# amberxie88/latent_diffusion_planning

Measured on AMD Instinct MI355X. Metric: latent plans/sec (horizon=9, 100 DDIM steps), higher is better.
Workload: dtype f32; 1 GPU; configs[1]: rm_lift planner ConditionalUnet1D (D=25, T=8, down_dims [256,512,1024]), 100-step DDIM, batch 256 synthetic latents per GPU, random-init weights, Philox noise, hipGraph-captured loop; plans_per_gpu=256, denoise_steps=100, sampler=ddim, graph=True, parallelism=dp1, ranks_seen_by_backend=1, backend=none, range_fallback=0, fp16_plane_launches=0

## Files before the change

### latent_diffusion_planning_amd/csrc/engine.hip

```cpp
#include "engine.hpp"
#include "sconv.hpp"
#include "t2pack.hpp"
#include "t4pack.hpp"
#include "version.h"

#include <algorithm>
#include <cmath>
#include <cstring>

namespace ldp {

void betas_squaredcos(int n, std::vector<float>& betas, std::vector<float>& alphas,
                             std::vector<float>& acp) {
  auto abar = [](double t) {
    const double c = std::cos((t + 0.008) / 1.008 * M_PI / 2.0);
    return c * c;
  };
  betas.resize(n);
  alphas.resize(n);
  acp.resize(n);
  float run = 1.0f;
  for (int i = 0; i < n; ++i) {
    const double b = std::min(1.0 - abar((double)(i + 1) / n) / abar((double)i / n), 0.999);
    betas[i] = (float)b;
// ... 1572 lines not shown
  return agent_sample_impl(h, obs_emb, obs_frames, obs_horizon, x_init, x_noise, a_init, a_noise, seed, row_offset, sampler, planner_steps,
                           idm_steps, x_out, plan_out, action_out, act_lo, act_hi, act_dim, act_mode, B, use_graph, stream, nullptr, &cs);
}

int ldp_agent_sample_guided(ldp_handle* h, const float* obs_emb, int32_t obs_frames, int32_t obs_horizon, const float* x_init,
                            const float* x_noise, const float* a_init, const float* a_noise, const float* target, const float* wg,
                            const float* anchor, const float* lam, const float* beta, const float* lo, const float* hi, const float* rho,
                            int32_t n_rho, uint64_t seed, int64_t row_offset, int32_t sampler, int32_t planner_steps, int32_t idm_steps,
                            float* x_out, float* plan_out, float* action_out, const float* act_lo, const float* act_hi, int32_t act_dim,
                            int32_t act_mode, int32_t B, int32_t use_graph, void* stream) {
  const GuideSpec gd{target, wg, anchor, lam, beta, lo, hi, rho, n_rho};
  return agent_sample_impl(h, obs_emb, obs_frames, obs_horizon, x_init, x_noise, a_init, a_noise, seed, row_offset, sampler, planner_steps,
                           idm_steps, x_out, plan_out, action_out, act_lo, act_hi, act_dim, act_mode, B, use_graph, stream, nullptr, nullptr,
                           &gd);
}

int ldp_policy_sample(ldp_handle* h, const float* obs_emb, int32_t obs_frames, int32_t obs_horizon, int32_t img_width,
                      const float* x_init, const float* x_noise, uint64_t seed, int64_t row_offset, int32_t sampler, int32_t n_steps,
                      float* action_out, const float* act_lo, const float* act_hi, int32_t act_dim, int32_t act_mode,
                      int32_t B, int32_t use_graph, void* stream) {
  if (!h || !obs_emb || !action_out || B <= 0) return fail(LDP_EINVAL, "bad argument");
  if (!h->pl.ready) return fail(LDP_ESTATE, "planner weights not finalized");
  PlannerState& P = h->pl;
  const int ah = h->cfg.action_horizon, A = P.D;
  if (obs_horizon <= 0 || obs_frames < obs_horizon || P.G <= 0 || P.G % obs_horizon != 0)
    return fail(LDP_EINVAL, "obs_horizon %d does not divide global_cond_dim %d (frames given: %d)", obs_horizon, P.G, obs_frames);
  const int E = P.G / obs_horizon;
  if (img_width < 0 || img_width > E) return fail(LDP_EINVAL, "img_width %d must lie in 0..%d (the per-frame width)", img_width, E);
  if (ah < 1 || ah > P.T) return fail(LDP_EINVAL, "action_horizon %d must be in 1..pred_horizon %d", ah, P.T);
  if (act_dim != 0 && (act_dim != 1 && act_dim != A)) return fail(LDP_EINVAL, "action bounds of length %d (A = %d)", act_dim, A);
  if (act_dim != 0 && (!act_lo || !act_hi)) return fail(LDP_EINVAL, "action bounds missing");
  if (!x_noise) {
    if (const int b1 = batch_split(h, B)) {
      const size_t xr = (size_t)P.T * A, ar = (size_t)ah * A;
      LDP_TRY(ldp_policy_sample(h, obs_emb, obs_frames, obs_horizon, img_width, x_init, nullptr, seed, row_offset, sampler, n_steps,
                                action_out, act_lo, act_hi, act_dim, act_mode, b1, use_graph, stream));
      const int64_t c1 = h->last_conv_launches, t1 = h->last_total_launches;
      const int r2 = ldp_policy_sample(h, obs_emb + (size_t)b1 * obs_frames * E, obs_frames, obs_horizon, img_width,
                                       x_init ? x_init + b1 * xr : nullptr, nullptr, seed, row_offset + b1, sampler, n_steps,
                                       action_out + b1 * ar, act_lo, act_hi, act_dim, act_mode, B - b1, use_graph, stream);
      h->last_conv_launches += c1; h->last_total_launches += t1;
      return r2;
    }
  }
  LDP_TRY(check_sampler(sampler, n_steps, P.n_train, "planner", h));
  LDP_TRY(entry_fault_check(h));
  hipStream_t s = (hipStream_t)stream;
  LDP_TRY(planner_workspace(h, B));
  h->last_conv_launches = h->last_total_launches = 0;
  LoopSpec L{n_steps, sampler, x_noise != nullptr && sampler == LDP_SAMPLER_DDPM, 0, n_steps};
  LDP_TRY(planner_pre(h, nullptr, x_init, x_noise, seed, row_offset, L, B, s));
  LDP_TRY(gather_dp_cond_launch(obs_emb, P.cond.f(), B, obs_frames, E, obs_horizon, img_width, s));
  const int Bg = bucket_rows(B, L.explicit_noise);
  GraphKey key{0, Bg, n_steps, sampler, L.explicit_noise ? 1 : 0, 0, 0, 0, n_steps};
  LDP_TRY(run_or_replay(h, key, use_graph != 0, s, [&](hipStream_t q) { return planner_loop(h, Bg, L, q); }));
  LDP_TRY(head_rows_launch(P.state.f(), action_out, B, P.T, ah, A, P.DP, s));
  if (act_dim != 0) LDP_TRY(normalize_launch(action_out, action_out, (int64_t)B * ah * A, act_lo, act_hi, act_dim, act_mode, s));
  return LDP_OK;
}

int ldp_normalize_bounds(const float* x, float* y, int64_t n, const float* lo, const float* hi,
                         int32_t dim, int32_t normalize, void* stream) {
  if (!x || !y || !lo || !hi || dim <= 0) return fail(LDP_EINVAL, "bad argument");
  return normalize_launch(x, y, n, lo, hi, dim, normalize, (hipStream_t)stream);
}

int ldp_mean_sq_diff(const float* a, const float* b, int64_t n, float* out, void* stream) {
  if (!a || !b || !out || n <= 0) return fail(LDP_EINVAL, "bad argument");
  return mean_sq_diff_launch(a, b, n, out, (hipStream_t)stream);
}

int ldp_reduce_stats(const float* x, int64_t n, float* out4, void* stream) {
  if (!x || !out4 || n <= 0) return fail(LDP_EINVAL, "bad argument");
  return reduce_stats_launch(x, n, out4, (hipStream_t)stream);
}

int ldp_add_noise(const float* x0, const float* noise, const int32_t* t_dev, int32_t n_train, float* out, int64_t rows,
                  int32_t width, void* stream) {
  if (!x0 || !noise || !t_dev || !out || rows <= 0 || width <= 0) return fail(LDP_EINVAL, "bad argument");
  if (n_train < 1 || n_train > 256) return fail(LDP_EINVAL, "n_train must be in 1..256 (the abar table travels by value), got %d", n_train);
  std::vector<float> betas, alphas, acp;
  betas_squaredcos(n_train, betas, alphas, acp);
  AbarTable tab{};
  std::copy(acp.begin(), acp.end(), tab.v);
  return add_noise_launch(x0, noise, t_dev, tab, n_train, out, rows, width, (hipStream_t)stream);
}

int ldp_check_fault(ldp_handle* h, void* stream) {
  if (!h) return fail(LDP_EINVAL, "null handle");
  LDP_HIP(hipStreamSynchronize((hipStream_t)stream));
  reap_retired_graphs(h);
  int32_t f = 0;
  LDP_TRY(ldp_poll_fault(h, &f));
  if (f & 1)
    return fail(LDP_EFAULT, "a split work-group timed out waiting for its peer: the results enqueued since the "
                "previous check are invalid (the handle now runs in safe mode; re-issue the calls)");
  if (f & 2)
    return fail(LDP_EFAULT, "an operand left the range of the two-fp16-plane form (|x| >= 65504): the results enqueued since the "
                "previous check are invalid (the handle now runs its split convolutions on three bf16 planes; re-issue the calls)");
  return LDP_OK;
}

int ldp_poll_fault(ldp_handle* h, int32_t* faulted) {
  if (!h || !faulted) return fail(LDP_EINVAL, "bad argument");
  const int f = h->fault_pending | take_faults(h);
  h->fault_pending = 0;
  *faulted = f;
  return LDP_OK;
}

int ldp_set_option(ldp_handle* h, const char* name, int64_t value) {
  if (!h || !name) return fail(LDP_EINVAL, "bad argument");
  const std::string n(name);
  Options& o = h->opt;
  const int v = (int)value;
  if (n == "no_csplit") o.no_csplit = v;
  else if (n == "no_mb2") o.no_mb2 = v;
  else if (n == "no_kw") o.no_kw = v;
  else if (n == "kw_min_it") o.kw_min_it = v;
  else if (n == "kw_bmax") o.kw_bmax = v;
  else if (n == "no_fin_rows") o.no_fin_rows = v;
  else if (n == "no_batch_split") o.no_batch_split = v;
  else if (n == "up_full_depth") o.up_full_depth = v;
  else if (n == "planner_split") o.planner_split = v;
  else if (n == "planner_split_updown") o.planner_split_updown = v;
  else if (n == "planner_split_cs2") o.planner_split_cs2 = v;
  else if (n == "planner_split_c256") o.planner_split_c256 = v;
  else if (n == "planner_split_mb2") o.planner_split_mb2 = v;
  else if (n == "planner_split_t2res") o.planner_split_t2res = v;
  else if (n == "planner_split_t16") o.planner_split_t16 = v;
  else if (n == "planner_split_f16") o.planner_split_f16 = v;
  else if (n == "vae_no_conv_stats") o.vae_no_conv_stats = v;
  else if (n == "vae_no_conv_in_stats") o.vae_no_conv_in_stats = v;
  else if (n == "vae_split") o.vae_split = v;
  else if (n == "vae_split_f16") o.vae_split_f16 = v;
  else if (n == "vae_split_gn_only") o.vae_split_gn_only = v;
  else if (n == "vae_split_s2") o.vae_split_s2 = v;
  else if (n == "graph_cap") { h->graph_cap = v; return LDP_OK; }
  else if (n == "timeline_ptr") o.timeline_ptr = value;
  else if (n == "idm_unfused") o.idm_unfused = v;
  else if (n == "idm_rt_major") o.idm_rt_major = v;
  else if (n == "idm_noring") o.idm_noring = v;
  else if (n == "idm_stream") o.idm_stream = v;
  else if (n == "by_sample") o.by_sample = v;
  else if (n == "place2d") { o.place2d = v; drop_graphs(h); }
  else if (n == "idm_f16") o.idm_f16 = v;
  else if (n == "idm_f16_min_rows") o.idm_f16_min_rows = v < 32 ? 32 : v;
  else if (n == "idm_f16_hs") o.idm_f16_hs = v;
  else if (n == "train_small_wg") o.train_small_wg = v;
  else if (n == "train_big") o.train_big = v;
  else if (n == "train_split") o.train_split = v;
  else if (n == "train_streams") o.train_streams = v;
  else if (n == "train_intra_split") o.train_intra_split = v;
  else if (n == "train_group_proj") o.train_group_proj = v;
  else if (n == "train_gn4") o.train_gn4 = v;
  else if (n == "train_sides") o.train_sides = v;
  else if (n == "train_fuse_reduce") o.train_fuse_reduce = v;
  else if (n == "train_wg_target") o.train_wg_target = v;
  else if (n == "idm_hs") { if (v != 0 && v != 1 && v != 2 && v != 4 && v != 8) return fail(LDP_EINVAL, "idm_hs must be 0, 1, 2, 4 or 8"); o.idm_hs = v; }
  else if (n == "dbg" || n == "repeat") {
#ifdef LDP_ABLATE
    if (n == "dbg") o.dbg = v; else o.repeat = v < 1 ? 1 : v;
#else
    if (!(n == "dbg" ? v == 0 : v == 1))
      return fail(LDP_EINVAL, "option '%s': the timing ablations are compiled into libldp_hip_abl.so only (make -C csrc ablate; tools take it with --lib)", name);
#endif
  }
  else if (n == "t2_mb2") o.t2_mb2 = v;
  else if (n == "planner_split_t2all16") o.planner_split_t2all16 = v;
  else if (n == "planner_split_t2res16") o.planner_split_t2res16 = v;
  else if (n == "planner_split_8w") o.planner_split_8w = v;
  else if (n == "safe_mode") h->safe_mode = v != 0;
  else if (n == "range_fallback") h->range_fallback = v != 0;
  else if (n == "dump_plans") {
    std::map<std::string, int64_t> text = v == 2 ? tconv_plan_log() : std::map<std::string, int64_t>();
    if (v != 2) for (const auto& kv : h->plan_log) text[plan_text(kv.first)] = kv.second;
    for (const auto& kv : text) fprintf(stderr, "PLAN %s launches=%lld\n", kv.first.c_str(), (long long)kv.second);
    return LDP_OK;
  }
  else if (n == "inject_fault") { if (v && h->fault_host) h->fault_host[v == 2 ? 1 : 0] = 1u; return LDP_OK; }
  else return fail(LDP_EKEY, "unknown option '%s'", name);
  drop_graphs(h);
  return LDP_OK;
}

int ldp_get_option(ldp_handle* h, const char* name, int64_t* value) {
  if (!h || !name || !value) return fail(LDP_EINVAL, "bad argument");
  const std::string n(name);
  const Options& o = h->opt;
  if (n == "no_csplit") *value = o.no_csplit;
  else if (n == "no_mb2") *value = o.no_mb2;
  else if (n == "no_kw") *value = o.no_kw;
  else if (n == "kw_min_it") *value = o.kw_min_it;
  else if (n == "kw_bmax") *value = o.kw_bmax;
  else if (n == "no_fin_rows") *value = o.no_fin_rows;
  else if (n == "no_batch_split") *value = o.no_batch_split;
  else if (n == "up_full_depth") *value = o.up_full_depth;
  else if (n == "planner_split") *value = o.planner_split;
  else if (n == "planner_split_updown") *value = o.planner_split_updown;
  else if (n == "planner_split_cs2") *value = o.planner_split_cs2;
  else if (n == "planner_split_c256") *value = o.planner_split_c256;
  else if (n == "planner_split_mb2") *value = o.planner_split_mb2;
  else if (n == "planner_split_t2res") *value = o.planner_split_t2res;
  else if (n == "planner_split_t16") *value = o.planner_split_t16;
  else if (n == "planner_split_f16") *value = o.planner_split_f16;
  else if (n == "stat_f16_launches") *value = h->stat_f16_launches;
  else if (n == "stat_t2_shared_launches") *value = h->stat_t2_shared_launches;
  else if (n == "stat_t4_shared_launches") *value = h->stat_t4_shared_launches;
  else if (n == "stat_mb2_launches") *value = h->stat_mb2_launches;
  else if (n.rfind("stat_train_gemm_", 0) == 0) {
    static const char* const forms[3] = {"nn", "nt", "tn"};
    static const char* const tiles[5] = {"32", "32_ki2", "64", "64_ki2", "128"};
    const std::string rest = n.substr(16);
    int idx = rest == "fused" ? LDP_STAT_GEMM_FUSED : rest == "reduce" ? LDP_STAT_GEMM_REDUCE : -1;
    for (int f = 0; f < 3 && idx < 0; ++f)
      for (int t = 0; t < 5; ++t)
        if (rest == std::string(forms[f]) + "_" + tiles[t]) idx = f * 5 + t;
    if (idx < 0) return fail(LDP_EKEY, "unknown option '%s'", name);
    *value = h->stat_train_gemm[idx];
  }
  else if (n.rfind("stat_idm_", 0) == 0) {
    const std::string rest = n.substr(9);
    int idx = rest == "unfused" ? LDP_STAT_IDM_UNFUSED : rest == "f16_hs2" ? LDP_STAT_IDM_F16_HS2 : rest == "f16_hs4" ? LDP_STAT_IDM_F16_HS4 : -1;
    for (int hs = 1; hs <= 8 && idx < 0; hs *= 2)
      for (int ring = 0; ring <= (hs >= 4 ? 1 : 0); ++ring)
        for (int nt = 0; nt < 2; ++nt)
          if (rest == "f32_hs" + std::to_string(hs) + (ring ? "_ring" : "") + (nt ? "_nt" : "")) idx = stat_idm_f32(hs, ring != 0, nt != 0);
    if (idx < 0) return fail(LDP_EKEY, "unknown option '%s'", name);
    *value = h->stat_idm[idx];
  }
  else if (n == "vae_no_conv_stats") *value = o.vae_no_conv_stats;
  else if (n == "vae_no_conv_in_stats") *value = o.vae_no_conv_in_stats;
  else if (n == "vae_split") *value = o.vae_split;
  else if (n == "vae_split_f16") *value = o.vae_split_f16;
  else if (n == "vae_split_gn_only") *value = o.vae_split_gn_only;
  else if (n == "vae_split_s2") *value = o.vae_split_s2;
  else if (n == "timeline_ptr") *value = o.timeline_ptr;
  else if (n == "idm_unfused") *value = o.idm_unfused;
  else if (n == "idm_rt_major") *value = o.idm_rt_major;
  else if (n == "idm_noring") *value = o.idm_noring;
  else if (n == "idm_stream") *value = o.idm_stream;
  else if (n == "by_sample") *value = o.by_sample;
  else if (n == "place2d") *value = o.place2d;
  else if (n == "idm_hs") *value = o.idm_hs;
  else if (n == "idm_f16") *value = o.idm_f16;
  else if (n == "idm_f16_min_rows") *value = o.idm_f16_min_rows;
  else if (n == "idm_f16_hs") *value = o.idm_f16_hs;
  else if (n == "train_small_wg") *value = o.train_small_wg;
  else if (n == "train_big") *value = o.train_big;
  else if (n == "train_split") *value = o.train_split;
  else if (n == "train_streams") *value = o.train_streams;
  else if (n == "train_intra_split") *value = o.train_intra_split;
  else if (n == "train_group_proj") *value = o.train_group_proj;
  else if (n == "train_gn4") *value = o.train_gn4;
  else if (n == "train_sides") *value = o.train_sides;
  else if (n == "train_fuse_reduce") *value = o.train_fuse_reduce;
  else if (n == "train_wg_target") *value = o.train_wg_target;
  else if (n == "dbg") *value = o.dbg;
  else if (n == "repeat") *value = o.repeat;
  else if (n == "t2_mb2") *value = o.t2_mb2;
  else if (n == "planner_split_t2all16") *value = o.planner_split_t2all16;
  else if (n == "planner_split_t2res16") *value = o.planner_split_t2res16;
  else if (n == "planner_split_8w") *value = o.planner_split_8w;
  else if (n == "safe_mode") *value = h->safe_mode ? 1 : 0;
  else if (n == "range_fallback") *value = h->range_fallback ? 1 : 0;
  else if (n == "range_faults_seen") *value = h->range_faults_seen;
  else if (n == "any_debug") *value = o.any_debug() ? 1 : 0;
  else if (n == "faults_seen") *value = h->faults_seen;
  else if (n == "n_cu") *value = h->n_cu;
  else if (n == "graphs") *value = (int64_t)h->graphs.size();
  else if (n == "graph_cap") *value = h->graph_cap;
  else if (n == "graphs_captured") *value = h->graphs_captured;
  else if (n == "graphs_evicted") *value = h->graphs_evicted;
  else return fail(LDP_EKEY, "unknown option '%s'", name);
  return LDP_OK;
}

int ldp_philox_raw(uint64_t seed, uint64_t elem0, uint32_t step, uint32_t stream_id, uint32_t* out_dev,
                   int64_t n, void* stream) {
  if (!out_dev || n <= 0) return fail(LDP_EINVAL, "bad argument");
  return philox_raw_launch(seed, elem0, step, stream_id, out_dev, n, (hipStream_t)stream);
}

int ldp_philox_normal(uint64_t seed, uint64_t elem0, uint32_t step, uint32_t stream_id, float* out_dev,
                      int64_t n, void* stream) {
  if (!out_dev || n <= 0) return fail(LDP_EINVAL, "bad argument");
  return philox_normal_launch(seed, elem0, step, stream_id, out_dev, n, (hipStream_t)stream);
}

int ldp_launch_count(ldp_handle* h, int32_t which, int64_t* launches) {
  if (!h || !launches) return fail(LDP_EINVAL, "bad argument");
  *launches = which == 0 ? h->last_conv_launches : h->last_total_launches;
  return LDP_OK;
}

static int prim_conv(int mode, const float* x, const float* kernel_host, const float* bias_host,
                     const float* gs, const float* gb, const float* film, float* y, int B, int t_in,
                     int cin, int cout, void* stream) {
  if (!x || !kernel_host || !bias_host || !y || B <= 0) return fail(LDP_EINVAL, "bad argument");
  hipStream_t s = (hipStream_t)stream;
  const int nj = mode_taps(mode);
  const int to = mode == MODE_DOWN ? t_in / 2 : mode == MODE_UP ? t_in * 2 : t_in;
  if (cout % 128 != 0) return fail(LDP_EINVAL, "Cout must be a multiple of 128 (8 groups x 16)");
  const int cin_p = round_up(cin, 32);
  ConvPlan p;
  LDP_TRY(pick_plan(mode, to, cout, cin_p, cin_p, false, p));
  const int cin_pp = round_up(cin_p, p.chunk());
  if (cin_pp != cin_p) LDP_TRY(pick_plan(mode, to, cout, cin_pp, cin_pp, false, p));
  std::vector<float> packed = t2_shared(mode, to, 0) ? pack_conv_t2(kernel_host, nullptr, cin, cout, cin_pp, cout)
                            : t4_shared(mode, to, 0) ? pack_conv_t4(kernel_host, nullptr, cin, cout, cin_pp, cout)
                                                     : pack_conv(kernel_host, nj, cin, cout, cin_pp, cout);
  DevBuf dw, db, dgs, dgb, dx, dfg, dft;
  LDP_TRY(upload(dw, packed.data(), packed.size() * 4, s));
  LDP_TRY(upload(db, bias_host, (size_t)cout * 4, s));
  ConvArgs a{};
  if (gs) {
    LDP_TRY(upload(dgs, gs, (size_t)cout * 4, s));
    LDP_TRY(upload(dgb, gb, (size_t)cout * 4, s));
    a.flags |= EP_GN;
  }
  const float* xin = x;
  if (cin_pp != cin) {
    LDP_TRY(dx.alloc((size_t)B * t_in * cin_pp * 4));
    LDP_TRY(pad_rows_launch(x, dx.f(), (int64_t)B * t_in, cin, cin_pp, s));
    xin = dx.f();
  }
  if (film) {
    LDP_TRY(dft.alloc((size_t)2 * cout * 4));
    LDP_HIP(hipMemsetAsync(dft.p, 0, (size_t)2 * cout * 4, s));
    a.film_t = dft.f(); a.film_g = film; a.film_stride = 2 * cout; a.flags |= EP_FILM;
  }
  a.xa = xin; a.ca = cin_pp; a.w = dw.f(); a.bias = db.f();
  a.gn_scale = dgs.f(); a.gn_bias = dgb.f();
  a.out = y; a.B = B; a.cout = cout; a.k = 0; a.rows_valid = B * to;
  const int r = tconv_launch(p, a, s);
  if (r != 0) return fail(r == -100 ? LDP_EINVAL : LDP_EHIP, "primitive conv launch failed (%d)", r);
  LDP_HIP(hipStreamSynchronize(s));
  return LDP_OK;
}

int ldp_conv1d_gn_mish_film_f32(const float* x, const float* kernel_host, const float* bias_host,
                                const float* gn_scale_host, const float* gn_bias_host,
                                const float* film, float* y, int32_t B, int32_t T, int32_t Cin,
                                int32_t Cout, void* stream) {
  if (!gn_scale_host || !gn_bias_host) return fail(LDP_EINVAL, "GroupNorm parameters required");
  return prim_conv(MODE_K5, x, kernel_host, bias_host, gn_scale_host, gn_bias_host, film, y, B, T, Cin,
                   Cout, stream);
}

int ldp_downsample1d_f32(const float* x, const float* kernel_host, const float* bias_host, float* y,
                         int32_t B, int32_t T, int32_t C, void* stream) {
  if (T % 2) return fail(LDP_EINVAL, "T must be even");
  return prim_conv(MODE_DOWN, x, kernel_host, bias_host, nullptr, nullptr, nullptr, y, B, T, C, C, stream);
}

int ldp_upsample1d_f32(const float* x, const float* kernel_host, const float* bias_host, float* y,
                       int32_t B, int32_t T, int32_t C, void* stream) {
  return prim_conv(MODE_UP, x, kernel_host, bias_host, nullptr, nullptr, nullptr, y, B, T, C, C, stream);
}

}
```

### latent_diffusion_planning_amd/csrc/tconv.hpp

```cpp
#pragma once
#include <hip/hip_runtime.h>
#include <stdint.h>
#include <type_traits>

#pragma clang fp contract(off)

#ifndef LDP_W_NT
#define LDP_W_NT 0
#endif
#ifndef LDP_SPLIT_NPROD
#define LDP_SPLIT_NPROD 6
#endif
#ifndef LDP_S16_LF
#define LDP_S16_LF 100
#endif
#ifndef LDP_F16_MINW
#define LDP_F16_MINW 2
#endif
#ifndef LDP_RANGE_GUARD
#define LDP_RANGE_GUARD 1
#endif
#ifndef LDP_KERNARG_TOUCH
#define LDP_KERNARG_TOUCH 1
#endif
// ... 810 lines not shown
          }
        }
      }
      if constexpr (T4F) {
#pragma unroll
        for (int m = 0; m < MB; ++m) {
          const f32x4 se0 = tit[m][0] + tit[m][1], se1 = tit[m][0] + tit[m][2];
          acc[m][0] = acc[m][0] + ((se0 + tit[m][3]) + tit[m][4]);
          acc[m][1] = acc[m][1] + ((se1 + tit[m][3]) + tit[m][5]);
          acc[m][2] = acc[m][2] + ((se0 + tit[m][6]) + tit[m][7]);
          acc[m][3] = acc[m][3] + ((se1 + tit[m][6]) + tit[m][8]);
        }
      }
    } else
    if (!dead_slice) {
#pragma unroll
    for (int ci = 0; ci < CPI; ++ci) {
#pragma unroll
      for (int s = 0; s < 4; ++s) {
#pragma unroll
        for (int j = 0; j < NJ; ++j) {
#pragma unroll
          for (int to = 0; to < TO; ++to) {
            const int ti = tap_src(MODE, to, j);
            if (ti >= 0 && ti < TI) {
#pragma unroll
              for (int m = 0; m < MB; ++m)
                acc[m][to] = __builtin_amdgcn_mfma_f32_16x16x4f32(areg[m][ti][ci][s], bc[j][ci][s],
                                                                  acc[m][to], 0, 0, 0);
            }
          }
        }
        if (RES_OUT) {
#pragma unroll
          for (int to = 0; to < TO; ++to)
#pragma unroll
            for (int m = 0; m < MB; ++m)
              racc[m][to] = __builtin_amdgcn_mfma_f32_16x16x4f32(areg[m][to][ci][s], rc[ci][s],
                                                                 racc[m][to], 0, 0, 0);
        }
      }
    }
    }
    if (LAST) {
#pragma unroll
      for (int i = 0; i < MBE * TI * CPI; ++i) __builtin_amdgcn_sched_group_barrier(0x100, 1, 0);
    } else {
      constexpr int NUSED = (tap_used(MODE, TO, 0) ? 1 : 0) + (NJ > 1 && tap_used(MODE, TO, 1) ? 1 : 0) +
                            (NJ > 2 && tap_used(MODE, TO, 2) ? 1 : 0) + (NJ > 3 && tap_used(MODE, TO, 3) ? 1 : 0) +
                            (NJ > 4 && tap_used(MODE, TO, 4) ? 1 : 0);
      constexpr int NLOADS = NLDE + ((T4S ? T4_SLOTS : NUSED) + (RES_OUT ? 1 : 0)) * CPI;
      constexpr int NMFMA = MBE * CPI * 4 * (conv_products(MODE, TO, SPLIT) + (RES_OUT ? TO : 0));
      constexpr int MPL = NMFMA / NLOADS > 0 ? NMFMA / NLOADS : 1;
#pragma unroll
      for (int i = 0; i < MBE * TI * CPI; ++i) __builtin_amdgcn_sched_group_barrier(0x100, 1, 0);
#pragma unroll
      for (int i = 0; i < NLOADS; ++i) {
        __builtin_amdgcn_sched_group_barrier(0x020, 1, 0);
        __builtin_amdgcn_sched_group_barrier(0x008, MPL, 0);
      }
      if (NMFMA - NLOADS * MPL > 0) __builtin_amdgcn_sched_group_barrier(0x008, NMFMA - NLOADS * MPL, 0);
      __builtin_amdgcn_sched_group_barrier(0x200, NLDE, 0);
    }
    if (!LAST) stage_store(pass_tag, xnext);
    __syncthreads();
  };

#define LDP_TCONV_PASS(pass_tag) \
  stage_load(pass_tag, it0); \
  wload(S16 ? it0 * NSTEP : it0, wb0, rb0); \
  stage_store(pass_tag, smem + (it0 & 1) * C::XT); \
  __syncthreads(); \
  LDP_TL(1); \
  if (mode_2d(MODE) && !S16) { \
    for (int it = it0; it < nit; it += 2) { \
      iteration(pass_tag, std::false_type{}, it, wb0, rb0, wb1, rb1); \
      if (it + 1 < nit) iteration(pass_tag, std::false_type{}, it + 1, wb1, rb1, wb0, rb0); \
    } \
  } else { \
    int it = it0; \
    if constexpr (S16 && NSTEP % 2 == 0) { \
      for (; it + 1 < nit; ++it) iteration(pass_tag, std::false_type{}, it, wb0, rb0, wb1, rb1); \
      iteration(pass_tag, std::true_type{}, it, wb0, rb0, wb1, rb1); \
    } else { \
    for (; it + 2 < nit; it += 2) { \
      iteration(pass_tag, std::false_type{}, it, wb0, rb0, wb1, rb1); \
      iteration(pass_tag, std::false_type{}, it + 1, wb1, rb1, wb0, rb0); \
    } \
    if (it + 2 == nit) { \
      iteration(pass_tag, std::false_type{}, it, wb0, rb0, wb1, rb1); \
      iteration(pass_tag, std::true_type{}, it + 1, wb1, rb1, wb0, rb0); \
    } else if (it + 1 == nit) { \
      iteration(pass_tag, std::true_type{}, it, wb0, rb0, wb1, rb1); \
    } \
    } \
  }
  auto t4_combine_pass = [&](auto pass_tag) {
  if constexpr (T4S && !T4F) {
    constexpr int PASS = decltype(pass_tag)::value;
#pragma unroll
    for (int mm = 0; mm < MBE; ++mm) {
      const int m = T4P ? PASS : mm;
      const f32x4 se0 = tacc[mm][0] + tacc[mm][1], se1 = tacc[mm][0] + tacc[mm][2];
      acc[m][0] = (se0 + tacc[mm][3]) + tacc[mm][4];
      acc[m][1] = (se1 + tacc[mm][3]) + tacc[mm][5];
      acc[m][2] = (se0 + tacc[mm][6]) + tacc[mm][7];
      acc[m][3] = (se1 + tacc[mm][6]) + tacc[mm][8];
#pragma unroll
      for (int k = 0; k < T4_SLOTS; ++k) tacc[mm][k] = f32x4{0.f, 0.f, 0.f, 0.f};
    }
  }
  };
  {
    using pass0 = std::integral_constant<int, 0>;
    LDP_TCONV_PASS(pass0{})
    t4_combine_pass(pass0{});
  }
  if constexpr (T4P) {
    using pass1 = std::integral_constant<int, 1>;
    LDP_TCONV_PASS(pass1{})
    t4_combine_pass(pass1{});
  }
#undef LDP_TCONV_PASS

  if constexpr (T2S) {
#pragma unroll
    for (int m = 0; m < MB; ++m) {
      if constexpr (T2S2) {
        sacc[m] = sacc[m] + sacc_b[m];
        acc[m][0] = acc[m][0] + acc_b[m][0];
        acc[m][1] = acc[m][1] + acc_b[m][1];
      }
      acc[m][0] = sacc[m] + acc[m][0];
      acc[m][1] = sacc[m] + acc[m][1];
    }
  }
  if constexpr (C::F16 && S32) {
#pragma unroll
    for (int t = 0; t < TO; ++t)
#pragma unroll
      for (int i = 0; i < 16; ++i) acc32[t][i] = acc32[t][i] + acc32_lo[t][i] * (1.0f / 2048.0f);
    if constexpr (RES_OUT) {
#pragma unroll
      for (int t = 0; t < TO; ++t)
#pragma unroll
        for (int i = 0; i < 16; ++i) racc32[t][i] = racc32[t][i] + racc32_lo[t][i] * (1.0f / 2048.0f);
    }
  }
  if constexpr (C::F16 && !S32) {
#pragma unroll
    for (int m = 0; m < MB; ++m) {
#pragma unroll
      for (int t = 0; t < TO; ++t) acc[m][t] = acc[m][t] + acc_lo[m][t] * (1.0f / 2048.0f);
      if constexpr (RES_OUT) {
#pragma unroll
        for (int t = 0; t < TO; ++t) racc[m][t] = racc[m][t] + racc_lo[m][t] * (1.0f / 2048.0f);
      }
    }
  }
  LDP_TL(2);
  if LDP_ABL(16) return;
  const int ecol = wn * 16 + (lane & 15);
  const int erow0 = (lane >> 4) * 4;
  const int flags = (a.flags & mode_flag_mask(MODE)) | mode_flag_forced(MODE);
  constexpr int EPL = C::EPL;
  constexpr int NS = 16 * MB;
  constexpr int SPW = (NS + C::NW - 1) / C::NW;
  constexpr bool FULL = (NS % C::NW) == 0;
  const unsigned lane_to = BN <= 64 ? (unsigned)lane / BN : 0u;
  const unsigned lane_col = BN <= 64 ? (unsigned)lane % BN : (unsigned)lane;
  auto e_to = [](int e) { return BN <= 64 ? e * (64 / BN) : e / (BN / 64); };
  auto e_col = [](int e) { return BN <= 64 ? 0 : 64 * (e % (BN / 64)); };
  const unsigned lane_chan = (unsigned)(cbk * BN) + lane_col;
  const unsigned lane_eoff = __umul24(lane_to, (unsigned)a.cout) + lane_chan;
  const unsigned lane_uoff = __umul24(lane_to, (unsigned)a.d_real) + lane_chan;
  float p_bias[EPL], p_gs[EPL], p_gb[EPL], p_rb[EPL];
  float p_fts[SPW][EPL], p_fgs[SPW][EPL], p_ftb[SPW][EPL], p_fgb[SPW][EPL], p_add[SPW][EPL], p_nz[SPW][EPL];
#pragma unroll
  for (int e = 0; e < EPL; ++e) {
    p_bias[e] = (a.bias + e_col(e))[lane_chan];
    p_gs[e] = (flags & EP_GN) ? (a.gn_scale + e_col(e))[lane_chan] : 1.0f;
    p_gb[e] = (flags & EP_GN) ? (a.gn_bias + e_col(e))[lane_chan] : 0.0f;
    p_rb[e] = RES_OUT ? (a.bres + e_col(e))[lane_chan] : 0.0f;
  }
  const bool f_film = (flags & EP_FILM) != 0, f_res = (flags & EP_RESIN) != 0;
  const bool f_step = (flags & EP_STEP) != 0;
#pragma unroll
  for (int si = 0; si < SPW; ++si)
#pragma unroll
    for (int e = 0; e < EPL; ++e) p_fts[si][e] = p_fgs[si][e] = p_ftb[si][e] = p_fgb[si][e] = p_add[si][e] = p_nz[si][e] = 0.0f;
  if (f_film) {
#pragma unroll
    for (int si = 0; si < SPW; ++si) {
      const int sr = wave + si * C::NW;
      const int b = (b0 + sr) < a.B ? (b0 + sr) : (a.B - 1);
      int kk = a.k;
      if (a.k_dev) kk = a.k_dev[b];
      const float* ft = a.film_t + (size_t)kk * a.film_stride;
      const float* fg = a.film_g + (size_t)b * a.film_stride;
#pragma unroll
      for (int e = 0; e < EPL; ++e) {
        p_fts[si][e] = (ft + e_col(e))[lane_chan];
        p_fgs[si][e] = (fg + e_col(e))[lane_chan];
        p_ftb[si][e] = (ft + a.cout + e_col(e))[lane_chan];
        p_fgb[si][e] = (fg + a.cout + e_col(e))[lane_chan];
      }
    }
  }
  if (f_res || f_step) {
    const float* rp = f_res ? a.res_in : a.out;
#pragma unroll
    for (int si = 0; si < SPW; ++si) {
      const int sr = wave + si * C::NW;
      const int b = (b0 + sr) < a.B ? (b0 + sr) : (a.B - 1);
#pragma unroll
      for (int e = 0; e < EPL; ++e)
        p_add[si][e] = (rp + ((size_t)b * TO + e_to(e)) * a.cout + e_col(e))[lane_eoff];
    }
  }
  if (f_step && a.noise && a.coef.sigma != 0.f) {
#pragma unroll
    for (int si = 0; si < SPW; ++si) {
      const int sr = wave + si * C::NW;
      const int b = (b0 + sr) < a.B ? (b0 + sr) : (a.B - 1);
#pragma unroll
      for (int e = 0; e < EPL; ++e) {
        const int to = (int)lane_to + e_to(e), c = (int)lane_chan + e_col(e);
        if (c < a.d_real && (b * TO + to) < a.rows_valid)
          p_nz[si][e] = (a.noise + ((size_t)b * TO + e_to(e)) * a.d_real + e_col(e))[lane_uoff];
      }
    }
  }

  {
    constexpr int pass = 0;
    if constexpr (S32) {
#pragma unroll
      for (int to = 0; to < TO; ++to)
#pragma unroll
        for (int i = 0; i < 16; ++i) {
          const int row32 = (i & 3) + 8 * (i >> 2) + 4 * (lane >> 5);
          smem[((((row32 >> 4) * KS + ks) * TO + to) * 16 + (row32 & 15)) * BNP + wn * 32 + (lane & 31)] = acc32[to][i];
        }
    } else
#pragma unroll
    for (int m = 0; m < MB; ++m) {
#pragma unroll
      for (int to = 0; to < TO; ++to) {
#pragma unroll
        for (int i = 0; i < 4; ++i)
          smem[(((m * KS + ks) * TO + to) * 16 + erow0 + i) * BNP + ecol] = acc[m][to][i];
      }
    }
    __syncthreads();
    LDP_TL(3);

    constexpr int TILE = NS * TO * BN;
    constexpr bool KW_OK = KWS && (MODE == MODE_K5 || MODE == MODE_DOWN || MODE == MODE_UP) && MB == 1 && TO * BN <= 512;
    unsigned long long* kw_tile = nullptr;
    unsigned int ktag = 0;
    if (KW_OK && kw > 1) {
      const int tile_id = sb * (ngroups * cs) + cbk;
      kw_tile = a.kw_slab + (size_t)(tile_id * kw) * (2 * TILE);
      ktag = (((unsigned int)a.ctl[2] & 0xfffu) << 20) | (((unsigned int)a.step + 1u) << 6) | (unsigned int)a.kw_slot;
      if (kpart != 0) {
        unsigned long long* mine = kw_tile + (size_t)kpart * (2 * TILE);
#pragma unroll
        for (int pass = 0; pass < (RES_OUT ? 2 : 1); ++pass) {
          if (pass == 1) {
            __syncthreads();
#pragma unroll
            for (int to = 0; to < TO; ++to)
#pragma unroll
              for (int i = 0; i < 4; ++i)
                smem[((ks * TO + to) * 16 + erow0 + i) * BNP + ecol] = racc[0][RES_OUT ? to : 0][i];
            __syncthreads();
          }
          const auto krsrc = __builtin_amdgcn_make_buffer_rsrc(mine, 0, 0x7ffffff0, 0x00020000);
          constexpr int PAIRS = TO * BN / 2;
#pragma unroll
          for (int si = 0; si < SPW; ++si) {
            const int sr = wave + si * C::NW;
            if (!FULL && sr >= NS) continue;
#pragma unroll
            for (int pc = 0; pc < (PAIRS + 63) / 64; ++pc) {
              if (PAIRS < 64 && lane >= PAIRS) continue;
              const int el = 2 * (lane + 64 * pc);
              const int to = el / BN, col = el % BN;
              float x0 = 0.0f, x1 = 0.0f;
#pragma unroll
              for (int k2 = 0; k2 < KS; ++k2) {
                x0 += smem[((k2 * TO + to) * 16 + sr) * BNP + col];
                x1 += smem[((k2 * TO + to) * 16 + sr) * BNP + col + 1];
              }
              const unsigned long long g0 = granule_pack(ktag, x0), g1 = granule_pack(ktag, x1);
              const u32x4_t gv = {(unsigned int)g0, (unsigned int)(g0 >> 32), (unsigned int)g1, (unsigned int)(g1 >> 32)};
              __builtin_amdgcn_raw_buffer_store_b128(gv, krsrc, (unsigned int)((pass * TILE + sr * (TO * BN) + el) * 8), 0, AUX_SC1);
            }
          }
        }
        return;
      }
    }
    auto kw_add = [&](float x, int pass, int sr, int el) {
      if (!(KW_OK && kw > 1)) return x;
      unsigned long long pv[KW_MAX - 1];
      int spin = 0;
      for (;;) {
        bool ok = true;
#pragma unroll
        for (int q = 0; q < KW_MAX - 1; ++q) {
          pv[q] = 0;
          if (q + 1 < kw)
            pv[q] = __hip_atomic_load(kw_tile + (size_t)(q + 1) * (2 * TILE) + pass * TILE + sr * (TO * BN) + el,
                                      __ATOMIC_RELAXED, __HIP_MEMORY_SCOPE_AGENT);
        }
        asm volatile("s_waitcnt vmcnt(0)" ::: "memory");
#pragma unroll
        for (int q = 0; q < KW_MAX - 1; ++q) ok = ok && (q + 1 >= kw || granule_ok(pv[q], ktag));
        if (__all(ok)) break;
        if (++spin > (1 << 18) || ((spin & 1023) == 0 && __hip_atomic_load(a.fault, __ATOMIC_RELAXED, __HIP_MEMORY_SCOPE_SYSTEM) != 0u)) {
          if (lane == 0) *a.fault = 1u;
          break;
        }
        __builtin_amdgcn_s_sleep(1);
      }
#pragma unroll
      for (int q = 0; q < KW_MAX - 1; ++q) x += (q + 1 < kw) ? __uint_as_float((unsigned int)pv[q]) : 0.0f;
      return x;
    };

    const bool xch = (cs > 1) && (flags & EP_GN) && !LDP_ABL(32);
    const auto xrsrc = __builtin_amdgcn_make_buffer_rsrc(const_cast<unsigned long long*>(a.xchg), 0, 0x7ffffff0, 0x00020000);
    unsigned int xbase = 0;
    unsigned int tag = 0;
    if (xch) {
      xbase = (unsigned int)((sb * MB * ngroups + grp) * 4) * 256u;
      tag = ((unsigned int)a.ctl[2] << 12) + (unsigned int)a.step + 1u;
    }
    float vv[SPW][EPL];
    float s1a[SPW], s2a[SPW];
    bool range_bad = false;
#pragma unroll
    for (int si = 0; si < SPW; ++si) {
      const int sr = wave + si * C::NW;
      float s1 = 0.f, s2 = 0.f;
#pragma unroll
      for (int e = 0; e < EPL; ++e) {
        const int el = lane + 64 * e;
        const int to = el / BN, col = el % BN;
        float x = p_bias[e];
        if (FULL || sr < NS) {
#pragma unroll
          for (int k2 = 0; k2 < KS; ++k2)
            x += smem[((((sr >> 4) * KS + k2) * TO + to) * 16 + (sr & 15)) * BNP + col];
          x = kw_add(x, 0, sr, el);
        }
        vv[si][e] = x;
        s1 += x;
        s2 += x * x;
      }
      if (flags & EP_GN) {
        s1 = wave_sum(s1);
        s2 = wave_sum(s2);
        if (xch && (FULL || sr < NS) && lane == 0) {
          const unsigned long long g1 = granule_pack(tag, s1), g2 = granule_pack(tag, s2);
          const u32x4_t gv = {(unsigned int)g1, (unsigned int)(g1 >> 32), (unsigned int)g2, (unsigned int)(g2 >> 32)};
          __builtin_amdgcn_raw_buffer_store_b128(gv, xrsrc, xbase + (unsigned int)(((sr >> 4) * ngroups * 4 + half) * 256 + (sr & 15) * 16), 0, AUX_SC1);
        }
      }
      if constexpr (C::F16) {
        if (LDP_RANGE_GUARD) range_bad = range_bad || !(s2 <= 3.0e38f);
      }
      s1a[si] = s1;
      s2a[si] = s2;
    }

    LDP_TL(4);
    if (RES_OUT) {
      __syncthreads();
      if constexpr (S32) {
#pragma unroll
        for (int to = 0; to < TO; ++to)
#pragma unroll
          for (int i = 0; i < 16; ++i) {
            const int row32 = (i & 3) + 8 * (i >> 2) + 4 * (lane >> 5);
            smem[((((row32 >> 4) * KS + ks) * TO + to) * 16 + (row32 & 15)) * BNP + wn * 32 + (lane & 31)] = racc32[RES_OUT ? to : 0][i];
          }
      } else
#pragma unroll
      for (int m = 0; m < MB; ++m) {
#pragma unroll
        for (int to = 0; to < TO; ++to) {
#pragma unroll
          for (int i = 0; i < 4; ++i)
            smem[(((m * KS + ks) * TO + to) * 16 + erow0 + i) * BNP + ecol] = racc[m][RES_OUT ? to : 0][i];
        }
      }
      __syncthreads();
#pragma unroll
      for (int si = 0; si < SPW; ++si) {
        const int sr = wave + si * C::NW;
        const int b = b0 + sr;
        if ((!FULL && sr >= NS) || b >= a.B) continue;
#pragma unroll
        for (int e = 0; e < EPL; ++e) {
          const int el = lane + 64 * e;
          const int to = el / BN, col = el % BN;
          float x = p_rb[e];
#pragma unroll
          for (int k2 = 0; k2 < KS; ++k2)
            x += smem[((((sr >> 4) * KS + k2) * TO + to) * 16 + (sr & 15)) * BNP + col];
          x = kw_add(x, 1, sr, el);
          if (!LDP_ABL(128) || x == 12345.f) (a.res_out + ((size_t)b * TO + e_to(e)) * a.cout + e_col(e))[lane_eoff] = x;
        }
      }
    }

    LDP_TL(5);
    float gs1 = 0.f, gs2 = 0.f;
#pragma unroll
    for (int si = 0; si < SPW; ++si) {
      const int sr = wave + si * C::NW;
      if (!FULL && sr >= NS) continue;
      const int b = b0 + sr;
      const bool live = b < a.B;
      float* v = vv[si];
      float mean = 0.f, rstd = 1.f;
      if (flags & EP_GN) {
        float s1 = s1a[si], s2 = s2a[si];
        if (xch) {
          u32x4_t pg[3];
          int spin = 0;
          for (;;) {
#pragma unroll
            for (int q = 0; q < 3; ++q) {
              pg[q] = u32x4_t{0u, 0u, 0u, 0u};
              if (q < cs - 1) {
                const int pp = q < half ? q : q + 1;
                pg[q] = __builtin_amdgcn_raw_buffer_load_b128(xrsrc, xbase + (unsigned int)(((sr >> 4) * ngroups * 4 + pp) * 256 + (sr & 15) * 16), 0, AUX_SC1);
              }
            }
            asm volatile("s_waitcnt vmcnt(0)" : "+v"(pg[0]), "+v"(pg[1]), "+v"(pg[2]) :: "memory");
            bool ok = true;
#pragma unroll
            for (int q = 0; q < 3; ++q)
              ok = ok && (q >= cs - 1 || (((pg[q][0] ^ pg[q][1]) == tag) && ((pg[q][2] ^ pg[q][3]) == tag)));
            if (ok) break;
            if (++spin > (1 << 20) || ((spin & 1023) == 0 && __hip_atomic_load(a.fault, __ATOMIC_RELAXED, __HIP_MEMORY_SCOPE_SYSTEM) != 0u)) {
              if (lane == 0) *a.fault = 1u;
              break;
            }
            __builtin_amdgcn_s_sleep(1);
          }
#ifdef LDP_TIMELINE
          if (a.tl && lane == 0) {
            atomicAdd(&a.tl[120000], 1ull);
            atomicAdd(&a.tl[120001], (unsigned long long)spin);
          }
#endif
          float t1 = 0.f, t2 = 0.f;
#pragma unroll
          for (int pp = 0; pp < 4; ++pp) {
            if (pp >= cs) continue;
            const int q = pp < half ? pp : pp - 1;
            float p1 = s1, p2 = s2;
            if (pp != half) {
              p1 = __uint_as_float(q == 0 ? pg[0][0] : q == 1 ? pg[1][0] : pg[2][0]);
              p2 = __uint_as_float(q == 0 ? pg[0][2] : q == 1 ? pg[1][2] : pg[2][2]);
            }
            t1 = pp == 0 ? p1 : t1 + p1;
            t2 = pp == 0 ? p2 : t2 + p2;
          }
          s1 = t1;
          s2 = t2;
        }
        const float inv_n = 1.0f / (float)(TO * BN * cs);
        mean = s1 * inv_n;
        const float var = fmaxf(s2 * inv_n - mean * mean, 0.0f);
#if LDP_EPILOGUE_IEEE
        rstd = 1.0f / sqrtf(var + 1e-6f);
#else
        rstd = __builtin_amdgcn_rsqf(var + 1e-6f);
#endif
      }
      if (!live) continue;
#pragma unroll
      for (int e = 0; e < EPL; ++e) {
        const int el = lane + 64 * e;
        const int to = el / BN, col = el % BN;
        const int c = cbk * BN + col;
        float y = v[e];
        if (flags & EP_GN) {
          y = (y - mean) * rstd * p_gs[e] + p_gb[e];
          y = mish_f(y);
        }
        if (flags & EP_FILM) y = (p_fts[si][e] + p_fgs[si][e]) * y + (p_ftb[si][e] + p_fgb[si][e]);
        float* const optr = a.out + ((size_t)b * TO + e_to(e)) * a.cout + e_col(e);
        if (flags & EP_RESIN) y += p_add[si][e];
        if (flags & EP_RELU) y = fmaxf(y, 0.0f);
        if (flags & (EP_STEP | EP_EPSOUT)) {
          if (c < a.d_real && (b * TO + to) < a.rows_valid) {
            if (flags & EP_EPSOUT) (a.eps_out + ((size_t)b * TO + e_to(e)) * a.d_real + e_col(e))[lane_uoff] = y;
            if (flags & EP_STEP) {
              const float xt = p_add[si][e];
              float z = 0.f;
              if (a.coef.sigma != 0.f) {
                if (a.noise) z = p_nz[si][e];
                else z = philox_normal(a.seed[0], (a.seed[1] + (uint64_t)(b * TO + to)) * (uint64_t)a.cout
                                       + (uint64_t)c, (uint32_t)a.step, 0u);
              }
              float x0 = (xt - a.coef.sqrt_1mab * y) * a.coef.inv_sqrt_ab;
              x0 = fminf(fmaxf(x0, -1.0f), 1.0f);
              optr[lane_eoff] = a.coef.c_x0 * x0 + a.coef.c_x * xt + a.coef.c_eps * y + a.coef.sigma * z;
            }
          }
        } else if (!LDP_ABL(128) || y == 12345.f) {
          optr[lane_eoff] = y;
          if (C::STATS) { gs1 += y; gs2 += y * y; }
        }
      }
    }
    if constexpr (C::F16) {
      if (LDP_RANGE_GUARD && range_bad && a.fault) a.fault[1] = 1u;
    }
    LDP_TL(6);
#ifdef LDP_TIMELINE
    if (a.tl) { asm volatile("s_waitcnt vmcnt(0)" ::: "memory"); LDP_TL(7); }
#endif
    if (C::STATS) {
      if (a.stats_part) {
        float* sp = smem + C::TILE_FLOATS;
        sp[wave * 64 + lane] = gs1;
        sp[(C::NW + wave) * 64 + lane] = gs2;
        __syncthreads();
        if (tid < 128) {
          const int which = tid >> 6, c = tid & 63;
          float t = 0.f;
#pragma unroll
          for (int w = 0; w < C::NW; ++w) t += sp[(which * C::NW + w) * 64 + c];
          a.stats_part[((size_t)sb * a.cout + cbk * BN + c) * 2 + which] = t;
        }
      }
    }
  }
}

__host__ __device__ constexpr bool tconv_kw_ok(int mode, int to, int nwn, int mb) {
  return (mode == MODE_K5 || mode == MODE_DOWN || mode == MODE_UP) && mb == 1 && to * 16 * nwn <= 512;
}

struct ConvPlan {
  int mode, to, nwn, ks, cpi, res_out;
  int mb = 1;
  int kws = 0;
  int split = 0;
  int bn() const { return 16 * nwn; }
  int chunk() const { return 16 * ks * cpi; }
};
int tconv_launch(const ConvPlan& p, const ConvArgs& a, hipStream_t stream);
int tconv_init_all();
int tconv_init_k5();
int tconv_init_k5r();
int tconv_init_misc();
int tconv_init_2d();
int tconv_launch_2d(const ConvPlan& p, const ConvArgs& a, hipStream_t stream);
int tconv_launch_k5(const ConvPlan& p, const ConvArgs& a, hipStream_t stream);
int tconv_launch_k5r(const ConvPlan& p, const ConvArgs& a, hipStream_t stream);
int tconv_launch_misc(const ConvPlan& p, const ConvArgs& a, hipStream_t stream);
int tconv_launch_split(const ConvPlan& p, const ConvArgs& a, hipStream_t stream);
int tconv_init_split();

}
```

Before: 5845 plans/s.

## Batch split-K polls and prefetch GroupNorm exchange partials across rows

Reworks the conv epilogue's cross-workgroup waits. Split-K partial polling now loads several elements per row in one wait loop instead of spinning per element. The GroupNorm stats-exchange poll uses one lane per peer with readlane and prefetches the next row's partials while the current row is normalized. Residual-output stores and the final stores are deferred into separate loops, which adds register pressure (rv array) and restructures the store ordering. A prim_conv padding-retry loop is also changed.

New measurement: 5911 plans/s, median of 6. 1.1% higher.

```diff
diff --git a/latent_diffusion_planning_amd/csrc/engine.hip b/latent_diffusion_planning_amd/csrc/engine.hip
--- a/latent_diffusion_planning_amd/csrc/engine.hip
+++ b/latent_diffusion_planning_amd/csrc/engine.hip
@@ -1898,11 +1898,12 @@
   const int nj = mode_taps(mode);
   const int to = mode == MODE_DOWN ? t_in / 2 : mode == MODE_UP ? t_in * 2 : t_in;
   if (cout % 128 != 0) return fail(LDP_EINVAL, "Cout must be a multiple of 128 (8 groups x 16)");
-  const int cin_p = round_up(cin, 32);
   ConvPlan p;
-  LDP_TRY(pick_plan(mode, to, cout, cin_p, cin_p, false, p));
-  const int cin_pp = round_up(cin_p, p.chunk());
-  if (cin_pp != cin_p) LDP_TRY(pick_plan(mode, to, cout, cin_pp, cin_pp, false, p));
+  int cin_pp = round_up(cin, 32);
+  for (int pad = 64; pick_plan(mode, to, cout, cin_pp, cin_pp, false, p) != LDP_OK; pad *= 2) {
+    if (pad > 256) return LDP_EINVAL;
+    cin_pp = round_up(cin, pad);
+  }
   std::vector<float> packed = t2_shared(mode, to, 0) ? pack_conv_t2(kernel_host, nullptr, cin, cout, cin_pp, cout)
                             : t4_shared(mode, to, 0) ? pack_conv_t4(kernel_host, nullptr, cin, cout, cin_pp, cout)
                                                      : pack_conv(kernel_host, nj, cin, cout, cin_pp, cout);
diff --git a/latent_diffusion_planning_amd/csrc/tconv.hpp b/latent_diffusion_planning_amd/csrc/tconv.hpp
--- a/latent_diffusion_planning_amd/csrc/tconv.hpp
+++ b/latent_diffusion_planning_amd/csrc/tconv.hpp
@@ -1136,32 +1136,41 @@
         return;
       }
     }
-    auto kw_add = [&](float x, int pass, int sr, int el) {
-      if (!(KW_OK && kw > 1)) return x;
-      unsigned long long pv[KW_MAX - 1];
-      int spin = 0;
-      for (;;) {
-        bool ok = true;
-#pragma unroll
-        for (int q = 0; q < KW_MAX - 1; ++q) {
-          pv[q] = 0;
-          if (q + 1 < kw)
-            pv[q] = __hip_atomic_load(kw_tile + (size_t)(q + 1) * (2 * TILE) + pass * TILE + sr * (TO * BN) + el,
-                                      __ATOMIC_RELAXED, __HIP_MEMORY_SCOPE_AGENT);
-        }
-        asm volatile("s_waitcnt vmcnt(0)" ::: "memory");
-#pragma unroll
-        for (int q = 0; q < KW_MAX - 1; ++q) ok = ok && (q + 1 >= kw || granule_ok(pv[q], ktag));
-        if (__all(ok)) break;
-        if (++spin > (1 << 18) || ((spin & 1023) == 0 && __hip_atomic_load(a.fault, __ATOMIC_RELAXED, __HIP_MEMORY_SCOPE_SYSTEM) != 0u)) {
-          if (lane == 0) *a.fault = 1u;
-          break;
-        }
-        __builtin_amdgcn_s_sleep(1);
-      }
-#pragma unroll
-      for (int q = 0; q < KW_MAX - 1; ++q) x += (q + 1 < kw) ? __uint_as_float((unsigned int)pv[q]) : 0.0f;
-      return x;
+    constexpr int KW_EC = EPL <= 2 ? EPL : 2;
+    auto kw_add_row = [&](float (&x)[EPL], int pass, int sr) {
+      if (!(KW_OK && kw > 1)) return;
+#pragma unroll
+      for (int e0 = 0; e0 < EPL; e0 += KW_EC) {
+        unsigned long long pv[KW_EC][KW_MAX - 1];
+        int spin = 0;
+        for (;;) {
+          bool ok = true;
+#pragma unroll
+          for (int e = 0; e < KW_EC; ++e)
+#pragma unroll
+            for (int q = 0; q < KW_MAX - 1; ++q) {
+              pv[e][q] = 0;
+              if (q + 1 < kw)
+                pv[e][q] = __hip_atomic_load(kw_tile + (size_t)(q + 1) * (2 * TILE) + pass * TILE + sr * (TO * BN) + lane + 64 * (e0 + e),
+                                             __ATOMIC_RELAXED, __HIP_MEMORY_SCOPE_AGENT);
+            }
+          asm volatile("s_waitcnt vmcnt(0)" ::: "memory");
+#pragma unroll
+          for (int e = 0; e < KW_EC; ++e)
+#pragma unroll
+            for (int q = 0; q < KW_MAX - 1; ++q) ok = ok && (q + 1 >= kw || granule_ok(pv[e][q], ktag));
+          if (__all(ok)) break;
+          if (++spin > (1 << 18) || ((spin & 1023) == 0 && __hip_atomic_load(a.fault, __ATOMIC_RELAXED, __HIP_MEMORY_SCOPE_SYSTEM) != 0u)) {
+            if (lane == 0) *a.fault = 1u;
+            break;
+          }
+          __builtin_amdgcn_s_sleep(1);
+        }
+#pragma unroll
+        for (int e = 0; e < KW_EC; ++e)
+#pragma unroll
+          for (int q = 0; q < KW_MAX - 1; ++q) x[e0 + e] += (q + 1 < kw) ? __uint_as_float((unsigned int)pv[e][q]) : 0.0f;
+      }
     };
 
     const bool xch = (cs > 1) && (flags & EP_GN) && !LDP_ABL(32);
@@ -1173,6 +1182,7 @@
       tag = ((unsigned int)a.ctl[2] << 12) + (unsigned int)a.step + 1u;
     }
     float vv[SPW][EPL];
+    float rv[SPW][EPL];
     float s1a[SPW], s2a[SPW];
     bool range_bad = false;
 #pragma unroll
@@ -1188,11 +1198,14 @@
 #pragma unroll
           for (int k2 = 0; k2 < KS; ++k2)
             x += smem[((((sr >> 4) * KS + k2) * TO + to) * 16 + (sr & 15)) * BNP + col];
-          x = kw_add(x, 0, sr, el);
         }
         vv[si][e] = x;
-        s1 += x;
-        s2 += x * x;
+      }
+      if (FULL || sr < NS) kw_add_row(vv[si], 0, sr);
+#pragma unroll
+      for (int e = 0; e < EPL; ++e) {
+        s1 += vv[si][e];
+        s2 += vv[si][e] * vv[si][e];
       }
       if (flags & EP_GN) {
         s1 = wave_sum(s1);
@@ -1236,103 +1249,149 @@
       for (int si = 0; si < SPW; ++si) {
         const int sr = wave + si * C::NW;
         const int b = b0 + sr;
+#pragma unroll
+        for (int e = 0; e < EPL; ++e) rv[si][e] = p_rb[e];
         if ((!FULL && sr >= NS) || b >= a.B) continue;
 #pragma unroll
         for (int e = 0; e < EPL; ++e) {
           const int el = lane + 64 * e;
           const int to = el / BN, col = el % BN;
-          float x = p_rb[e];
 #pragma unroll
           for (int k2 = 0; k2 < KS; ++k2)
-            x += smem[((((sr >> 4) * KS + k2) * TO + to) * 16 + (sr & 15)) * BNP + col];
-          x = kw_add(x, 1, sr, el);
-          if (!LDP_ABL(128) || x == 12345.f) (a.res_out + ((size_t)b * TO + e_to(e)) * a.cout + e_col(e))[lane_eoff] = x;
-        }
+            rv[si][e] += smem[((((sr >> 4) * KS + k2) * TO + to) * 16 + (sr & 15)) * BNP + col];
+        }
+        kw_add_row(rv[si], 1, sr);
       }
     }
 
     LDP_TL(5);
+    const int pq_pp = lane < half ? lane : lane + 1;
+    auto poll_issue = [&](int si, u32x4_t& pg) {
+      const int sr = wave + si * C::NW;
+      if (lane < cs - 1 && (FULL || sr < NS))
+        pg = __builtin_amdgcn_raw_buffer_load_b128(xrsrc, xbase + (unsigned int)(((sr >> 4) * ngroups * 4 + pq_pp) * 256 + (sr & 15) * 16), 0, AUX_SC1);
+    };
+    auto poll_wait = [&](int si, u32x4_t& pg) {
+      const int sr = wave + si * C::NW;
+      const bool pact = lane < cs - 1 && (FULL || sr < NS);
+      int spin = 0;
+      for (;;) {
+        asm volatile("s_waitcnt vmcnt(0)" : "+v"(pg) :: "memory");
+        const bool ok = !pact || (((pg[0] ^ pg[1]) == tag) && ((pg[2] ^ pg[3]) == tag));
+        if (__all(ok)) break;
+        if (++spin > (1 << 20) || ((spin & 1023) == 0 && __hip_atomic_load(a.fault, __ATOMIC_RELAXED, __HIP_MEMORY_SCOPE_SYSTEM) != 0u)) {
+          if (lane == 0) *a.fault = 1u;
+          break;
+        }
+        __builtin_amdgcn_s_sleep(1);
+        poll_issue(si, pg);
+      }
+#ifdef LDP_TIMELINE
+      if (a.tl && lane == 0) {
+        atomicAdd(&a.tl[120000], 1ull);
+        atomicAdd(&a.tl[120001], (unsigned long long)spin);
+      }
+#endif
+    };
+    u32x4_t pg_cur = {0u, 0u, 0u, 0u}, pg_nxt = {0u, 0u, 0u, 0u};
+    if (xch) {
+      poll_issue(0, pg_cur);
+      poll_wait(0, pg_cur);
+    }
+    LDP_TL(6);
+    auto settle = [](float& x) { asm volatile("" : "+v"(x)); };
+    if constexpr (SPW > 1 && SPW * EPL <= 4) {
+#pragma unroll
+      for (int e = 0; e < EPL; ++e) { settle(p_gs[e]); settle(p_gb[e]); }
+#pragma unroll
+      for (int si = 0; si < SPW; ++si)
+#pragma unroll
+        for (int e = 0; e < EPL; ++e) { settle(p_fts[si][e]); settle(p_fgs[si][e]); settle(p_ftb[si][e]); settle(p_fgb[si][e]); settle(p_add[si][e]); }
+    }
+
     float gs1 = 0.f, gs2 = 0.f;
 #pragma unroll
     for (int si = 0; si < SPW; ++si) {
       const int sr = wave + si * C::NW;
-      if (!FULL && sr >= NS) continue;
+      if (xch && si + 1 < SPW) poll_issue(si + 1, pg_nxt);
+      if (FULL || sr < NS) {
+        const int b = b0 + sr;
+        const bool live = b < a.B;
+        float* v = vv[si];
+        float mean = 0.f, rstd = 1.f;
+        if (flags & EP_GN) {
+          float s1 = s1a[si], s2 = s2a[si];
+          if (xch) {
+            float t1 = 0.f, t2 = 0.f;
+#pragma unroll
+            for (int pp = 0; pp < 4; ++pp) {
+              if (pp >= cs) continue;
+              const int q = pp < half ? pp : pp - 1;
+              float p1 = s1, p2 = s2;
+              if (pp != half) {
+                p1 = __uint_as_float(__builtin_amdgcn_readlane(pg_cur[0], q));
+                p2 = __uint_as_float(__builtin_amdgcn_readlane(pg_cur[2], q));
+              }
+              t1 = pp == 0 ? p1 : t1 + p1;
+              t2 = pp == 0 ? p2 : t2 + p2;
+            }
+            s1 = t1;
+            s2 = t2;
+          }
+          const float inv_n = 1.0f / (float)(TO * BN * cs);
+          mean = s1 * inv_n;
+          const float var = fmaxf(s2 * inv_n - mean * mean, 0.0f);
+#if LDP_EPILOGUE_IEEE
+          rstd = 1.0f / sqrtf(var + 1e-6f);
+#else
+          rstd = __builtin_amdgcn_rsqf(var + 1e-6f);
+#endif
+        }
+        if (live) {
+#pragma unroll
+          for (int e = 0; e < EPL; ++e) {
+            float y = v[e];
+            if (flags & EP_GN) {
+              y = (y - mean) * rstd * p_gs[e] + p_gb[e];
+              y = mish_f(y);
+            }
+            if (flags & EP_FILM) y = (p_fts[si][e] + p_fgs[si][e]) * y + (p_ftb[si][e] + p_fgb[si][e]);
+            if (flags & EP_RESIN) y += p_add[si][e];
+            if (flags & EP_RELU) y = fmaxf(y, 0.0f);
+            v[e] = y;
+          }
+        }
+      }
+      if (xch && si + 1 < SPW) {
+        poll_wait(si + 1, pg_nxt);
+        pg_cur = pg_nxt;
+      }
+    }
+    if (RES_OUT) {
+#pragma unroll
+      for (int si = 0; si < SPW; ++si) {
+        const int sr = wave + si * C::NW;
+        const int b = b0 + sr;
+        if ((!FULL && sr >= NS) || b >= a.B) continue;
+#pragma unroll
+        for (int e = 0; e < EPL; ++e) {
+          const float x = rv[si][e];
+          if (!LDP_ABL(128) || x == 12345.f) (a.res_out + ((size_t)b * TO + e_to(e)) * a.cout + e_col(e))[lane_eoff] = x;
+        }
+      }
+    }
+#pragma unroll
+    for (int si = 0; si < SPW; ++si) {
+      const int sr = wave + si * C::NW;
       const int b = b0 + sr;
-      const bool live = b < a.B;
-      float* v = vv[si];
-      float mean = 0.f, rstd = 1.f;
-      if (flags & EP_GN) {
-        float s1 = s1a[si], s2 = s2a[si];
-        if (xch) {
-          u32x4_t pg[3];
-          int spin = 0;
-          for (;;) {
-#pragma unroll
-            for (int q = 0; q < 3; ++q) {
-              pg[q] = u32x4_t{0u, 0u, 0u, 0u};
-              if (q < cs - 1) {
-                const int pp = q < half ? q : q + 1;
-                pg[q] = __builtin_amdgcn_raw_buffer_load_b128(xrsrc, xbase + (unsigned int)(((sr >> 4) * ngroups * 4 + pp) * 256 + (sr & 15) * 16), 0, AUX_SC1);
-              }
-            }
-            asm volatile("s_waitcnt vmcnt(0)" : "+v"(pg[0]), "+v"(pg[1]), "+v"(pg[2]) :: "memory");
-            bool ok = true;
-#pragma unroll
-            for (int q = 0; q < 3; ++q)
-              ok = ok && (q >= cs - 1 || (((pg[q][0] ^ pg[q][1]) == tag) && ((pg[q][2] ^ pg[q][3]) == tag)));
-            if (ok) break;
-            if (++spin > (1 << 20) || ((spin & 1023) == 0 && __hip_atomic_load(a.fault, __ATOMIC_RELAXED, __HIP_MEMORY_SCOPE_SYSTEM) != 0u)) {
-              if (lane == 0) *a.fault = 1u;
-              break;
-            }
-            __builtin_amdgcn_s_sleep(1);
-          }
-#ifdef LDP_TIMELINE
-          if (a.tl && lane == 0) {
-            atomicAdd(&a.tl[120000], 1ull);
-            atomicAdd(&a.tl[120001], (unsigned long long)spin);
-          }
-#endif
-          float t1 = 0.f, t2 = 0.f;
-#pragma unroll
-          for (int pp = 0; pp < 4; ++pp) {
-            if (pp >= cs) continue;
-            const int q = pp < half ? pp : pp - 1;
-            float p1 = s1, p2 = s2;
-            if (pp != half) {
-              p1 = __uint_as_float(q == 0 ? pg[0][0] : q == 1 ? pg[1][0] : pg[2][0]);
-              p2 = __uint_as_float(q == 0 ? pg[0][2] : q == 1 ? pg[1][2] : pg[2][2]);
-            }
-            t1 = pp == 0 ? p1 : t1 + p1;
-            t2 = pp == 0 ? p2 : t2 + p2;
-          }
-          s1 = t1;
-          s2 = t2;
-        }
-        const float inv_n = 1.0f / (float)(TO * BN * cs);
-        mean = s1 * inv_n;
-        const float var = fmaxf(s2 * inv_n - mean * mean, 0.0f);
-#if LDP_EPILOGUE_IEEE
-        rstd = 1.0f / sqrtf(var + 1e-6f);
-#else
-        rstd = __builtin_amdgcn_rsqf(var + 1e-6f);
-#endif
-      }
-      if (!live) continue;
+      if ((!FULL && sr >= NS) || b >= a.B) continue;
 #pragma unroll
       for (int e = 0; e < EPL; ++e) {
         const int el = lane + 64 * e;
         const int to = el / BN, col = el % BN;
         const int c = cbk * BN + col;
-        float y = v[e];
-        if (flags & EP_GN) {
-          y = (y - mean) * rstd * p_gs[e] + p_gb[e];
-          y = mish_f(y);
-        }
-        if (flags & EP_FILM) y = (p_fts[si][e] + p_fgs[si][e]) * y + (p_ftb[si][e] + p_fgb[si][e]);
+        const float y = vv[si][e];
         float* const optr = a.out + ((size_t)b * TO + e_to(e)) * a.cout + e_col(e);
-        if (flags & EP_RESIN) y += p_add[si][e];
-        if (flags & EP_RELU) y = fmaxf(y, 0.0f);
         if (flags & (EP_STEP | EP_EPSOUT)) {
           if (c < a.d_real && (b * TO + to) < a.rows_valid) {
             if (flags & EP_EPSOUT) (a.eps_out + ((size_t)b * TO + e_to(e)) * a.d_real + e_col(e))[lane_uoff] = y;
@@ -1358,9 +1417,16 @@
     if constexpr (C::F16) {
       if (LDP_RANGE_GUARD && range_bad && a.fault) a.fault[1] = 1u;
     }
-    LDP_TL(6);
 #ifdef LDP_TIMELINE
-    if (a.tl) { asm volatile("s_waitcnt vmcnt(0)" ::: "memory"); LDP_TL(7); }
+    if (a.tl) {
+      const unsigned long long t_issued = __builtin_amdgcn_s_memtime();
+      asm volatile("s_waitcnt vmcnt(0)" ::: "memory");
+      const unsigned long long t_landed = __builtin_amdgcn_s_memtime();
+      const unsigned long long drain = t_landed - t_issued < 0xffffull ? t_landed - t_issued : 0xffffull;
+      if (lane == 0)
+        a.tl[((size_t)(blockIdx.x + gridDim.x * (blockIdx.y + gridDim.y * blockIdx.z)) * 16 + wave) * 8 + 7] =
+            (t_landed & 0xffffffffffffull) | (drain << 48);
+    }
 #endif
     if (C::STATS) {
       if (a.stats_part) {
```
